# facebookresearch/multihop_dense_retrieval

Hardware: AMD Instinct MI355X
Metric: queries/sec (2-hop, beam-size x topk) over 5Mx768 index (higher is better)
Workload: dtype f32 (index stored as fp16 hi/lo pairs, fp32 accumulate); encoder f16 MFMA / f32 accumulate

## Files before the change

multihop_dense_retrieval_amd/csrc/mdr_encoder.hip:

```cpp
#include <hip/hip_runtime.h>
#include <map>
#include <mutex>
#include <algorithm>
#include <type_traits>

#include <cmath>
#include <cstdlib>
#include <cstring>
#include <new>
#include <string>
#include <vector>

#include "mdr_common.h"
#include "../../include/mdr_reader.h"

namespace mdr {
namespace {

#include "mdr_encoder_pack_ln.inl"
#include "mdr_encoder_gemm.inl"
#include "mdr_encoder_gemm_quad.inl"
#include "mdr_encoder_attention.inl"

}
}

using namespace mdr;

#ifndef MDR_CU_LANES
#define MDR_CU_LANES 0
#endif

namespace {

template <int EPI, typename C>
int launch_gemm_cfg(const _Float16* A, int lda, const _Float16* W, const float* bias, int M_cap, const int* M_dev, int N, int K, void* out, int ldo,
                    const _Float16* res, int ldr, hipStream_t st) {
    { int rc_ = ensure_dynamic_lds((const void*)gemm_f16_kernel<EPI, C>, C::LDS_BYTES); if (rc_) return rc_; }
    const int blocks = (N / C::BN) * ((M_cap + C::BM - 1) / C::BM);
    hipLaunchKernelGGL((gemm_f16_kernel<EPI, C>), dim3(blocks), dim3(C::THREADS), C::LDS_BYTES, st, A, lda, W, bias, M_cap, M_dev, N, K, out, ldo, res, ldr);
    MDR_HIP_TRY(hipGetLastError());
    return MDR_OK;
}

inline int persistent_rounds(int M_est, int bm, int N, int bn, int wgs_per_xcd) {
    const long long T = (long long)((M_est + bm - 1) / bm) * (N / bn);
    const long long per_xcd = (T + 7) / 8;
    return (int)((per_xcd + wgs_per_xcd - 1) / wgs_per_xcd);
}

template <int EPI, typename C>
int launch_gemm_persist(const _Float16* A, int lda, const _Float16* W, const float* bias, int M_cap, const int* M_dev, int N, int K, void* out, int ldo,
                        int M_est, int num_cus, hipStream_t st) {
    constexpr int lds = C::LDS_BYTES + kPersistBiasMax * 4;
    { int rc_ = ensure_dynamic_lds((const void*)gemm_persist_kernel<EPI, C>, lds); if (rc_) return rc_; }
    const int grid = num_cus / 8 * 8;
    hipLaunchKernelGGL((gemm_persist_kernel<EPI, C>), dim3(grid), dim3(C::THREADS), lds, st, A, lda, W, bias, M_cap, M_dev, N, K, out, ldo,
                       MDR_GEMM_EPI);
    MDR_HIP_TRY(hipGetLastError());
    return MDR_OK;
}

template <int EPI>
int launch_gemm_big(const _Float16* A, int lda, const _Float16* W, const float* bias, int M_cap, const int* M_dev, int N, int K, void* out, int ldo,
                    int M_est, int num_cus, hipStream_t st) {
    constexpr int lds = GemmB2::LDS_BYTES + kPersistBiasMax * 4 + 8 * 2048;
    const int grid = num_cus / 8 * 8;
    { int rc_ = ensure_dynamic_lds((const void*)gemm_big_kernel<EPI>, lds); if (rc_) return rc_; }
    hipLaunchKernelGGL((gemm_big_kernel<EPI>), dim3(grid), dim3(512), lds, st, A, lda, W, bias, M_cap, M_dev, N, K, out, ldo);
    MDR_HIP_TRY(hipGetLastError());
    return MDR_OK;
}

template <int EPI>
int launch_gemm_quad(const _Float16* A, int lda, const _Float16* W, const float* bias, int M_cap, const int* M_dev, int N, int K, void* out, int ldo,
                     int M_est, int num_cus, hipStream_t st) {
    constexpr int lds = GemmB2::LDS_BYTES + kPersistBiasMax * 4 + 4 * 4096;
    const int grid = num_cus / 8 * 8;
    { int rc_ = ensure_dynamic_lds((const void*)gemm_quad_kernel<EPI>, lds); if (rc_) return rc_; }
    hipLaunchKernelGGL((gemm_quad_kernel<EPI>), dim3(grid), dim3(256), lds, st, A, lda, W, bias, M_cap, M_dev, N, K, out, ldo);
    MDR_HIP_TRY(hipGetLastError());
    return MDR_OK;
}

template <int EPI>
int launch_gemm(const _Float16* A, int lda, const _Float16* W, const float* bias, int M_cap, const int* M_dev, int N, int K, void* out, int ldo,
                const _Float16* res, int ldr, int M_est, int num_cus, hipStream_t st, bool* res_added = nullptr, int force = -1) {
    static int env_sel = getenv("MDR_GEMM_CFG") ? atoi(getenv("MDR_GEMM_CFG")) : 0;
    int sel = force >= 0 ? force : env_sel;
    if (force < 0 && (sel == 4 || sel == 6 || sel == 7) && (long long)(N / 128) * ((M_est + 255) / 256) < (long long)num_cus * 3 / 2) sel = 0;
    if (res_added) *res_added = true;
    const long long p_tiles = (long long)(N / 128) * ((M_est + 255) / 256);
    if ((sel == 4 || sel == 6 || sel == 7 || (sel == 0 && p_tiles >= (long long)num_cus * 3 / 2)) && N % 128 == 0 && N <= kPersistBiasMax) {
        if (res_added) *res_added = false;
        else if (EPI == EPI_BIAS_RES_F32) return set_error(MDR_E_STATE, "large-M GEMM with a residual needs the caller to take the residual (res_added)");
        constexpr int E = EPI == EPI_BIAS_RES_F32 ? EPI_BIAS_F32 : EPI;
        const bool out32 = ((unsigned long long)M_cap + 255ull) * (unsigned long long)ldo * (E == EPI_BIAS_F32 ? 4ull : 2ull) < (1ull << 32);
        const bool a32 = ((unsigned long long)M_cap + 255ull) * (unsigned long long)lda * 2ull < (1ull << 32);
        if (sel == 7 && out32 && a32 && N % 256 == 0 && K % 128 == 0 && K >= 256) return launch_gemm_quad<E>(A, lda, W, bias, M_cap, M_dev, N, K, out, ldo, M_est, num_cus, st);
        if ((sel == 6 || sel == 0) && N % 256 == 0 && out32) {
            const double osz = (E == EPI_BIAS_F32) ? 4.0 : 2.0;
            const int grid = num_cus / 8 * 8, ntm_all = (M_est + 255) / 256;
            auto cost256 = [&](int max_rem, int tiles_per_pass, int* rounds_out) {
                const int head = gemm_head_row_tiles(ntm_all, N / 256, grid, max_rem);
                const int rounds = persistent_rounds(std::min(M_est, head * 256), 256, N, 256, num_cus / 8);
                const long long tail_tiles = (long long)((std::max(0, M_est - head * 256) + 127) / 128) * (N / 128);
                const long long passes = (tail_tiles + (long long)grid * tiles_per_pass - 1) / ((long long)grid * tiles_per_pass);
                if (rounds_out) *rounds_out = rounds;
                return rounds * ((256.0 + 256.0) * K * 2 + 256.0 * 256.0 * osz) + passes * 1.2 * ((128.0 + 128.0) * K * 2 + 128.0 * 128.0 * osz);
            };
            int rounds_q = 0;
            const double c_quad = cost256(grid / 4, 1, &rounds_q), c_big = cost256(grid / 2, 1, nullptr);
            const double c_p = persistent_rounds(M_est, 256, N, 128, num_cus / 8) * ((256.0 + 128.0) * K * 2 + 256.0 * 128.0 * osz);
            if (sel == 6 || std::min(c_big, c_quad) < c_p) {
                if (sel == 0 && a32 && K % 128 == 0 && K >= 256 && (rounds_q == 1 || K >= 2048) && c_quad <= 1.15 * c_big)
                    return launch_gemm_quad<E>(A, lda, W, bias, M_cap, M_dev, N, K, out, ldo, M_est, num_cus, st);
                return launch_gemm_big<E>(A, lda, W, bias, M_cap, M_dev, N, K, out, ldo, M_est, num_cus, st);
            }
        }
        return launch_gemm_persist<E, GemmP>(A, lda, W, bias, M_cap, M_dev, N, K, out, ldo, M_est, num_cus, st);
    }
    const long long big_blocks = (N % 256 == 0) ? (long long)(N / 256) * ((M_est + 255) / 256) : 0;
    const long long mid_blocks = (long long)(N / 128) * ((M_est + 127) / 128);
    const long long small_blocks = (long long)(N / 64) * ((M_est + 63) / 64);
    if (sel == 3 && big_blocks > 0) return launch_gemm_cfg<EPI, GemmBig>(A, lda, W, bias, M_cap, M_dev, N, K, out, ldo, res, ldr, st);
#ifdef MDR_GEMM_EXTRA_CFGS
    if (sel == 8) return launch_gemm_cfg<EPI, GemmCfg<128, 64, 2, 2, 3>>(A, lda, W, bias, M_cap, M_dev, N, K, out, ldo, res, ldr, st);
    if (sel == 9) return launch_gemm_cfg<EPI, GemmCfg<64, 128, 2, 2, 3>>(A, lda, W, bias, M_cap, M_dev, N, K, out, ldo, res, ldr, st);
    if (sel == 10) return launch_gemm_cfg<EPI, GemmCfg<128, 128, 2, 2, 3>>(A, lda, W, bias, M_cap, M_dev, N, K, out, ldo, res, ldr, st);
    if (sel == 11) return launch_gemm_cfg<EPI, GemmCfg<64, 64, 2, 2, 4>>(A, lda, W, bias, M_cap, M_dev, N, K, out, ldo, res, ldr, st);
    if (sel == 12) return launch_gemm_cfg<EPI, GemmCfg<128, 64, 4, 2, 3>>(A, lda, W, bias, M_cap, M_dev, N, K, out, ldo, res, ldr, st);
    if (sel == 13) return launch_gemm_cfg<EPI, GemmCfg<64, 64, 4, 2, 3>>(A, lda, W, bias, M_cap, M_dev, N, K, out, ldo, res, ldr, st);
#endif
    const long long c_mid = (mid_blocks + num_cus - 1) / num_cus * 256, c_small = (small_blocks + num_cus - 1) / num_cus * 128;
    if (N % 128 == 0 && (sel == 2 || (sel == 0 && c_mid < c_small)))
        return launch_gemm_cfg<EPI, GemmMid>(A, lda, W, bias, M_cap, M_dev, N, K, out, ldo, res, ldr, st);
    return launch_gemm_cfg<EPI, GemmSmall>(A, lda, W, bias, M_cap, M_dev, N, K, out, ldo, res, ldr, st);
}

template <int NT>
int launch_attention(const _Float16* qkv, const int* cu, int B, int L, int H, int heads, _Float16* ctx, hipStream_t st) {
    constexpr int lds = attention_lds_bytes<NT>();
    { int rc_ = ensure_dynamic_lds((const void*)attention_kernel<NT>, lds); if (rc_) return rc_; }
    dim3 grid(heads, B);
    hipLaunchKernelGGL((attention_kernel<NT>), grid, dim3(512), lds, st, qkv, cu, H, ctx);
    MDR_HIP_TRY(hipGetLastError());
    return MDR_OK;
}

int launch_attention_ring(const _Float16* qkv, const int* cu, const int* order, int B, int L, int H, int heads, _Float16* ctx, hipStream_t st) {
    { int rc_ = ensure_dynamic_lds((const void*)attention_ring_kernel, kRingLds); if (rc_) return rc_; }
    const int nblk = (L + 127) / 128;
    const long long pairs8 = ((long long)B * heads + 7) / 8 * 8;
    hipLaunchKernelGGL(attention_ring_kernel, dim3((unsigned)(pairs8 * nblk)), dim3(512), kRingLds, st, qkv, cu, order, B, heads, nblk, H, ctx);
    MDR_HIP_TRY(hipGetLastError());
    return MDR_OK;
}

template <int NTC>
int launch_attention_stream(const _Float16* qkv, const int* cu, const int* order, int B, int L, int H, int heads, _Float16* ctx, hipStream_t st) {
    if (MDR_ATTN_RING) return launch_attention_ring(qkv, cu, order, B, L, H, heads, ctx, st);
    constexpr int lds = NTC * 16 * 128 * 2;
    { int rc_ = ensure_dynamic_lds((const void*)attention_stream_kernel<NTC>, lds); if (rc_) return rc_; }
    dim3 grid(heads, B, (L + 127) / 128);
    hipLaunchKernelGGL((attention_stream_kernel<NTC>), grid, dim3(kAttnThreads), lds, st, qkv, cu, H, ctx);
    MDR_HIP_TRY(hipGetLastError());
    return MDR_OK;
}

constexpr int kOneShotMaxL = 32 * 16;
int launch_attention_for(int sel, const _Float16* qkv, const int* cu, const int* order, int B, int L, int H, int heads, _Float16* ctx, hipStream_t st) {
    if (sel == 2 || (sel == 0 && L > 128))
        return L <= 64 ? launch_attention_stream<4>(qkv, cu, order, B, L, H, heads, ctx, st) : launch_attention_stream<16>(qkv, cu, order, B, L, H, heads, ctx, st);
    if (L <= 128) return launch_attention<8>(qkv, cu, B, L, H, heads, ctx, st);
    if (L <= 384) return launch_attention<24>(qkv, cu, B, L, H, heads, ctx, st);
    return launch_attention<32>(qkv, cu, B, L, H, heads, ctx, st);
}

}

#include "mdr_encoder_trunk.inl"

struct mdr_encoder {
    Trunk t;
    _Float16* wproj = nullptr;
    float *bproj = nullptr, *lnp_g = nullptr, *lnp_b = nullptr;
    float fill_hint = 0.f;
};

namespace {

void launch_embed_ln(const long long* ids, const int* tok_src, const int* tok_pid, const int* total, int cap, const float* word, const float* pos,
                     const float* type0, const float* g, const float* b, int H, int vocab, int max_pos, float eps, _Float16* out16, float* out32,
                     hipStream_t st) {
    hipLaunchKernelGGL(embed_ln_kernel, dim3((cap + 3) / 4), dim3(256), 0, st, ids, tok_src, tok_pid, total, word, pos, type0, g, b, H, vocab, max_pos, eps,
                       out16, out32);
}

}

extern "C" {

int mdr_encoder_create(const mdr_encoder_config* cfg, const mdr_tensor* tensors, int n_tensors, int weights_on_device, int device, void* stream,
                       mdr_encoder** out) {
    MDR_REQUIRE(cfg && tensors && out, "NULL argument");
    MDR_REQUIRE(cfg->max_pos > 2, "bad geometry");
    if (int rc = trunk_check(*cfg, device)) return rc;
    DeviceGuard guard(device);
    mdr_encoder* h = new (std::nothrow) mdr_encoder();
    MDR_REQUIRE(h != nullptr, "out of host memory");
    const size_t H = cfg->hidden;
    WeightLoader ld{tensors, n_tensors, weights_on_device, (hipStream_t)stream, &h->t.allocs};
    trunk_upload(h->t, *cfg, device, 1, ld);
    ld.keep16("project.0.weight", H * H, &h->wproj);
    ld.keep32("project.0.bias", H, &h->bproj);
    ld.keep32("project.1.weight", H, &h->lnp_g);
    ld.keep32("project.1.bias", H, &h->lnp_b);
    if (int rc = ld.finish()) {
        mdr_encoder_free(h);
        return rc;
    }
    *out = h;
    return MDR_OK;
}

int mdr_test_gemm_f16(const void* A_dev, const void* W_dev, const float* bias_dev, int M, const int* m_dev, int N, int K, void* out_dev, int epilogue,
                      int kernel, int device, void* stream) {
    MDR_REQUIRE(A_dev && W_dev && bias_dev && out_dev, "NULL pointer");
    MDR_REQUIRE(M > 0 && N > 0 && K > 0 && N % 64 == 0 && K % 64 == 0, "bad GEMM shape M=%d N=%d K=%d (N, K multiples of 64)", M, N, K);
    MDR_REQUIRE(epilogue == EPI_BIAS_F16 || epilogue == EPI_BIAS_GELU_F16 || epilogue == EPI_BIAS_F32, "epilogue must be 0, 1 or 3");
#ifdef MDR_GEMM_EXTRA_CFGS
    MDR_REQUIRE(kernel == 0 || kernel == 1 || kernel == 2 || kernel == 4 || kernel == 6 || kernel == 7 || (kernel >= 8 && kernel <= 13), "kernel must be 0, 1, 2, 4, 6, 7 or 8-13");
#else
    MDR_REQUIRE(kernel == 0 || kernel == 1 || kernel == 2 || kernel == 4 || kernel == 6 || kernel == 7, "kernel must be 0, 1, 2, 4, 6 or 7");
#endif
    DeviceGuard guard(device);
    if (!guard.ok) return set_error(MDR_E_HIP, "hipSetDevice(%d) failed", device);
    const int ncu = device_cu_count(device);
    const _Float16* A = (const _Float16*)A_dev;
    const _Float16* W = (const _Float16*)W_dev;
    hipStream_t st = (hipStream_t)stream;
    if (epilogue == EPI_BIAS_F16) return launch_gemm<EPI_BIAS_F16>(A, K, W, bias_dev, M, m_dev, N, K, out_dev, N, nullptr, 0, M, ncu, st, nullptr, kernel);
    if (epilogue == EPI_BIAS_GELU_F16) return launch_gemm<EPI_BIAS_GELU_F16>(A, K, W, bias_dev, M, m_dev, N, K, out_dev, N, nullptr, 0, M, ncu, st, nullptr, kernel);
    return launch_gemm<EPI_BIAS_F32>(A, K, W, bias_dev, M, m_dev, N, K, out_dev, N, nullptr, 0, M, ncu, st, nullptr, kernel);
}

int mdr_test_gemm_ex(const void* A_dev, const void* W_dev, const float* bias_dev, const void* res16_dev, int M, int M_est, const int* m_dev, int N, int K,
                     void* out_dev, int epilogue, int kernel, int* res_added_host, int device, void* stream) {
    MDR_REQUIRE(A_dev && W_dev && bias_dev && out_dev, "NULL pointer");
    MDR_REQUIRE(M > 0 && N > 0 && K > 0 && N % 64 == 0 && K % 64 == 0, "bad GEMM shape M=%d N=%d K=%d (N, K multiples of 64)", M, N, K);
    MDR_REQUIRE(M_est >= 1, "M_est=%d must be at least 1", M_est);
    MDR_REQUIRE(epilogue >= EPI_BIAS_F16 && epilogue <= EPI_BIAS_F32, "epilogue must be 0, 1, 2 or 3");
    MDR_REQUIRE((epilogue == EPI_BIAS_RES_F32) == (res16_dev != nullptr), "res16_dev goes with epilogue 2 and with no other");
    MDR_REQUIRE(kernel == 0 || kernel == 1 || kernel == 2 || kernel == 4 || kernel == 6 || kernel == 7, "kernel must be 0, 1, 2, 4, 6 or 7");
    DeviceGuard guard(device);
    if (!guard.ok) return set_error(MDR_E_HIP, "hipSetDevice(%d) failed", device);
    const int ncu = device_cu_count(device);
    const _Float16* A = (const _Float16*)A_dev;
    const _Float16* W = (const _Float16*)W_dev;
    const _Float16* res = (const _Float16*)res16_dev;
    hipStream_t st = (hipStream_t)stream;
    bool added = true;
    bool* ra = res_added_host ? &added : nullptr;
    int rc;
    if (epilogue == EPI_BIAS_F16) rc = launch_gemm<EPI_BIAS_F16>(A, K, W, bias_dev, M, m_dev, N, K, out_dev, N, nullptr, 0, M_est, ncu, st, ra, kernel);
    else if (epilogue == EPI_BIAS_GELU_F16) rc = launch_gemm<EPI_BIAS_GELU_F16>(A, K, W, bias_dev, M, m_dev, N, K, out_dev, N, nullptr, 0, M_est, ncu, st, ra, kernel);
    else if (epilogue == EPI_BIAS_RES_F32) rc = launch_gemm<EPI_BIAS_RES_F32>(A, K, W, bias_dev, M, m_dev, N, K, out_dev, N, res, N, M_est, ncu, st, ra, kernel);
    else rc = launch_gemm<EPI_BIAS_F32>(A, K, W, bias_dev, M, m_dev, N, K, out_dev, N, nullptr, 0, M_est, ncu, st, ra, kernel);
    if (res_added_host) *res_added_host = added ? 1 : 0;
    return rc;
}

int mdr_test_attention(const void* qkv_dev, const int* cu_dev, const int* order_dev, int B, int L, int hidden, int heads, int kernel, void* ctx_dev,
                       int device, void* stream) {
    MDR_REQUIRE(qkv_dev && cu_dev && ctx_dev, "NULL pointer");
    MDR_REQUIRE(B >= 1, "B=%d must be at least 1", B);
    MDR_REQUIRE(L >= 1 && L <= 512, "L=%d out of range (1..512)", L);
    MDR_REQUIRE(heads >= 1 && hidden == 64 * heads, "head dim must be 64 (hidden=%d heads=%d)", hidden, heads);
    MDR_REQUIRE(kernel >= 0 && kernel <= 3, "kernel must be 0, 1, 2 or 3");
    MDR_REQUIRE(kernel != 1 || L <= kOneShotMaxL, "kernel 1 (one-shot) holds at most %d keys, L=%d", kOneShotMaxL, L);
    DeviceGuard guard(device);
    if (!guard.ok) return set_error(MDR_E_HIP, "hipSetDevice(%d) failed", device);
    const _Float16* qkv = (const _Float16*)qkv_dev;
    hipStream_t st = (hipStream_t)stream;
    if (kernel == 3) {
        hipLaunchKernelGGL(attention_cls_kernel, dim3(heads, B), dim3(64), 0, st, qkv, cu_dev, hidden, (_Float16*)ctx_dev);
        MDR_HIP_TRY(hipGetLastError());
        return MDR_OK;
    }
    return launch_attention_for(kernel, qkv, cu_dev, order_dev, B, L, hidden, heads, (_Float16*)ctx_dev, st);
}

#if MDR_GEMM_ABL == 5
int mdr_test_gemm_stamps(unsigned long long* out8_host, int reset) {
    MDR_REQUIRE(out8_host, "NULL pointer");
    MDR_HIP_TRY(hipDeviceSynchronize());
    MDR_HIP_TRY(hipMemcpyFromSymbol(out8_host, HIP_SYMBOL(g_gemm_stamp), 8 * sizeof(unsigned long long)));
    if (reset) {
        const unsigned long long z[8] = {0, 0, 0, 0, 0, 0, 0, 0};
        MDR_HIP_TRY(hipMemcpyToSymbol(HIP_SYMBOL(g_gemm_stamp), z, sizeof(z)));
    }
    return MDR_OK;
}
#endif

#if MDR_ATTN_ABL == 9
int mdr_test_attn_stamps(unsigned long long* out_host, int max_wgs) {
    MDR_REQUIRE(out_host && max_wgs > 0 && max_wgs <= kAttnStampWgs, "NULL pointer or max_wgs out of range");
    MDR_HIP_TRY(hipDeviceSynchronize());
    MDR_HIP_TRY(hipMemcpyFromSymbol(out_host, HIP_SYMBOL(g_attn_stamp), (size_t)max_wgs * 8 * sizeof(unsigned long long)));
    return MDR_OK;
}
#endif

#if MDR_CU_LANES
static std::mutex g_cu_mu;
static std::map<hipStream_t, int> g_stream_cus;
int mdr_stream_create_cu_range(int device, int cu_lo, int cu_hi, void** stream_out) {
    MDR_REQUIRE(stream_out != nullptr, "stream_out is NULL");
    DeviceGuard guard(device);
    if (!guard.ok) return set_error(MDR_E_HIP, "hipSetDevice(%d) failed", device);
    hipDeviceProp_t prop;
    MDR_HIP_TRY(hipGetDeviceProperties(&prop, device));
    const int n = prop.multiProcessorCount;
    MDR_REQUIRE(cu_lo >= 0 && cu_hi <= n && cu_hi - cu_lo >= 8 && cu_lo % 8 == 0 && cu_hi % 8 == 0, "CU range [%d, %d) must be multiples of 8 inside [0, %d)", cu_lo,
                cu_hi, n);
    std::vector<uint32_t> mask((size_t)(n + 31) / 32, 0u);
    for (int i = cu_lo; i < cu_hi; ++i) mask[(size_t)i / 32] |= 1u << (i % 32);
    hipStream_t st = nullptr;
    MDR_HIP_TRY(hipExtStreamCreateWithCUMask(&st, (uint32_t)mask.size(), mask.data()));
    *stream_out = (void*)st;
    return MDR_OK;
}

int mdr_stream_destroy(void* stream) {
    {
        std::lock_guard<std::mutex> lk(g_cu_mu);
        g_stream_cus.erase((hipStream_t)stream);
    }
    if (stream) MDR_HIP_TRY(hipStreamDestroy((hipStream_t)stream));
    return MDR_OK;
}
#endif

int mdr_encoder_set_fill_hint(mdr_encoder* h, float fill) {
    MDR_REQUIRE(h != nullptr, "encoder handle is NULL");
    MDR_REQUIRE(fill >= 0.f && fill <= 1.f, "fill must be in [0, 1] (0 = unknown)");
    h->fill_hint = fill;
    return MDR_OK;
}

int mdr_encoder_free(mdr_encoder* h) {
    if (!h) return MDR_OK;
    trunk_free(h->t);
    delete h;
    return MDR_OK;
}

size_t mdr_encoder_workspace_bytes(const mdr_encoder* h, int batch, int seq_len) {
    if (!h || batch <= 0 || seq_len <= 0) return 0;
    return carve(h->t.cfg, batch, seq_len, nullptr).bytes;
}

int mdr_encoder_forward(mdr_encoder* h, const int64_t* ids_dev, const int64_t* mask_dev, int batch, int seq_len, float* out_dev, void* workspace_dev,
                        size_t workspace_bytes, void* stream) {
    MDR_REQUIRE(h != nullptr, "encoder handle is NULL");
    MDR_REQUIRE(batch >= 0 && seq_len > 0, "bad shape batch=%d seq_len=%d", batch, seq_len);
    if (batch == 0) return MDR_OK;
    MDR_REQUIRE(ids_dev && mask_dev && out_dev, "NULL pointer");
    MDR_REQUIRE(seq_len <= 512, "seq_len=%d exceeds 512 (RoBERTa has 514 positions)", seq_len);
    MDR_REQUIRE((long long)batch * seq_len < (1ll << 31), "batch*seq_len overflows int32; split the batch");
    const Trunk& t = h->t;
    const mdr_encoder_config& c = t.cfg;
    DeviceGuard guard(t.device);
    hipStream_t st = (hipStream_t)stream;
    const long long* ids = (const long long*)ids_dev;
    Workspace w;
    if (int rc = trunk_begin(t, ids, (const long long*)mask_dev, batch, seq_len, workspace_dev, workspace_bytes, carve(c, batch, seq_len, nullptr).bytes, st, &w))
        return rc;
    const int B = batch, L = seq_len, H = c.hidden;
    const int Tcap = B * L;
    const int Test = h->fill_hint > 0.f ? std::max(1, (int)(h->fill_hint * (float)Tcap)) : Tcap - Tcap / 3;
    int ncu = t.num_cus;
#if MDR_CU_LANES
    {
        std::lock_guard<std::mutex> lk(g_cu_mu);
        auto it = g_stream_cus.find(st);
        if (it != g_stream_cus.end()) ncu = it->second;
        else {
            uint32_t mask[32] = {0};
            int n = 0;
            hipStreamCaptureStatus cs = hipStreamCaptureStatusNone;
            if (hipStreamIsCapturing(st, &cs) == hipSuccess && cs == hipStreamCaptureStatusNone && hipExtStreamGetCUMask(st, 32, mask) == hipSuccess)
                for (uint32_t w_ : mask) n += __builtin_popcount(w_);
            else (void)hipGetLastError();
            if (n >= 8 && n < t.num_cus) ncu = n / 8 * 8;
            if (cs == hipStreamCaptureStatusNone) g_stream_cus[st] = ncu;
        }
    }
#endif
    launch_embed_ln(ids, w.tok_src, w.tok_pid, w.total, Tcap, t.word, t.pos, t.type, t.emb_g, t.emb_b, H, c.vocab, c.max_pos, c.ln_eps, w.h16, w.h32, st);
    MDR_HIP_TRY(hipGetLastError());
    const Rows tokens{w.h16, w.h32, w.pre, Tcap, w.total, Test}, cls{w.cls16, w.cls32, w.clspre, B, nullptr, B};
    int rc;
    for (int i = 0; i + 1 < c.layers; ++i) {
        rc = trunk_layer(t, t.layers[i], w, tokens, B, L, ncu, st);
        if (rc) return rc;
    }
    const Layer& last = t.layers.back();
    rc = launch_qkv(t, last, w, tokens, ncu, st);
    if (rc) return rc;
    launch_gather_cls(w.h16, w.h32, w.cu, B, H, w.cls16, w.cls32, st);
    hipLaunchKernelGGL(attention_cls_kernel, dim3(c.heads, B), dim3(64), 0, st, (const _Float16*)w.qkv, (const int*)w.cu, H, w.ctx);
    MDR_HIP_TRY(hipGetLastError());
    rc = layer_tail(t, last, w.ctx, w.ffn, cls, ncu, st);
    if (rc) return rc;
    rc = launch_gemm<EPI_BIAS_F32>(w.cls16, H, h->wproj, h->bproj, B, nullptr, H, H, w.clspre, H, nullptr, 0, B, ncu, st);
    if (rc) return rc;
    launch_layernorm((const float*)w.clspre, (const _Float16*)nullptr, (const float*)nullptr, B, (const int*)nullptr, H, h->lnp_g, h->lnp_b, c.ln_eps,
                     (_Float16*)nullptr, out_dev, st);
    MDR_HIP_TRY(hipGetLastError());
    return MDR_OK;
}

}

#include "mdr_reader.inl"
#include "mdr_reader_assemble.inl"
#include "mdr_encoder_test_rows.inl"
#include "mdr_linear_grad.inl"
```

Measured before the change: 14830.

## Compute last-layer Q only for CLS rows and add tiny-M GEMM path

In the final encoder layer, only K and V are projected for all tokens. Q is computed just for the gathered CLS rows through a separate small GEMM, and the CLS attention kernel takes a separate Q pointer and stride. This removes the Q third of the last layer's QKV projection across all tokens. A GemmTiny configuration is also selected automatically for very small M. The diff references launch_kv, w.qcls, GemmTiny and kGemmSelTiny, none of which are defined in the visible changes, so it depends on edits to other files.

```diff
diff --git a/include/mdr_encoder_tail.h b/include/mdr_encoder_tail.h
--- /dev/null
+++ b/include/mdr_encoder_tail.h
@@ -0,0 +1,17 @@
+#ifndef MDR_ENCODER_TAIL_H
+#define MDR_ENCODER_TAIL_H
+
+#include "mdr_hip.h"
+
+#ifdef __cplusplus
+extern "C" {
+#endif
+
+int mdr_test_attention_cls(const void* q_dev, const void* qkv_dev, const int* cu_dev, int B, int hidden, int heads, void* ctx_dev, int device,
+                           void* stream);
+
+#ifdef __cplusplus
+}
+#endif
+
+#endif
diff --git a/multihop_dense_retrieval_amd/csrc/mdr_encoder.hip b/multihop_dense_retrieval_amd/csrc/mdr_encoder.hip
--- a/multihop_dense_retrieval_amd/csrc/mdr_encoder.hip
+++ b/multihop_dense_retrieval_amd/csrc/mdr_encoder.hip
@@ -13,6 +13,7 @@
 
 #include "mdr_common.h"
 #include "../../include/mdr_reader.h"
+#include "../../include/mdr_encoder_tail.h"
 
 namespace mdr {
 namespace {
@@ -120,6 +121,8 @@
         }
         return launch_gemm_persist<E, GemmP>(A, lda, W, bias, M_cap, M_dev, N, K, out, ldo, M_est, num_cus, st);
     }
+    if ((sel == kGemmSelTiny || (sel == 0 && M_cap <= kGemmTinyMaxRows && M_est <= kGemmTinyMaxRows)) && K % (BK * GemmTiny::KSUB) == 0)
+        return launch_gemm_cfg<EPI, GemmTiny>(A, lda, W, bias, M_cap, M_dev, N, K, out, ldo, res, ldr, st);
     const long long big_blocks = (N % 256 == 0) ? (long long)(N / 256) * ((M_est + 255) / 256) : 0;
     const long long mid_blocks = (long long)(N / 128) * ((M_est + 127) / 128);
     const long long small_blocks = (long long)(N / 64) * ((M_est + 63) / 64);
@@ -164,6 +167,13 @@
     { int rc_ = ensure_dynamic_lds((const void*)attention_stream_kernel<NTC>, lds); if (rc_) return rc_; }
     dim3 grid(heads, B, (L + 127) / 128);
     hipLaunchKernelGGL((attention_stream_kernel<NTC>), grid, dim3(kAttnThreads), lds, st, qkv, cu, H, ctx);
+    MDR_HIP_TRY(hipGetLastError());
+    return MDR_OK;
+}
+
+int launch_attention_cls(const _Float16* q, int ldq, int q_by_cu, const _Float16* qkv, const int* cu, int B, int H, int heads, _Float16* ctx_cls,
+                         hipStream_t st) {
+    hipLaunchKernelGGL(attention_cls_kernel, dim3(heads, B), dim3(64), 0, st, q, ldq, q_by_cu, qkv, cu, H, ctx_cls);
     MDR_HIP_TRY(hipGetLastError());
     return MDR_OK;
 }
@@ -252,7 +262,8 @@
     MDR_REQUIRE(M_est >= 1, "M_est=%d must be at least 1", M_est);
     MDR_REQUIRE(epilogue >= EPI_BIAS_F16 && epilogue <= EPI_BIAS_F32, "epilogue must be 0, 1, 2 or 3");
     MDR_REQUIRE((epilogue == EPI_BIAS_RES_F32) == (res16_dev != nullptr), "res16_dev goes with epilogue 2 and with no other");
-    MDR_REQUIRE(kernel == 0 || kernel == 1 || kernel == 2 || kernel == 4 || kernel == 6 || kernel == 7, "kernel must be 0, 1, 2, 4, 6 or 7");
+    MDR_REQUIRE(kernel == 0 || kernel == 1 || kernel == 2 || kernel == 4 || kernel == 6 || kernel == 7 || kernel == kGemmSelTiny,
+                "kernel must be 0, 1, 2, 4, 6, 7 or 16");
     DeviceGuard guard(device);
     if (!guard.ok) return set_error(MDR_E_HIP, "hipSetDevice(%d) failed", device);
     const int ncu = device_cu_count(device);
@@ -283,12 +294,20 @@
     if (!guard.ok) return set_error(MDR_E_HIP, "hipSetDevice(%d) failed", device);
     const _Float16* qkv = (const _Float16*)qkv_dev;
     hipStream_t st = (hipStream_t)stream;
-    if (kernel == 3) {
-        hipLaunchKernelGGL(attention_cls_kernel, dim3(heads, B), dim3(64), 0, st, qkv, cu_dev, hidden, (_Float16*)ctx_dev);
-        MDR_HIP_TRY(hipGetLastError());
-        return MDR_OK;
-    }
+    if (kernel == 3)
+        return launch_attention_cls(qkv, 3 * hidden, 1, qkv, cu_dev, B, hidden, heads, (_Float16*)ctx_dev, st);
     return launch_attention_for(kernel, qkv, cu_dev, order_dev, B, L, hidden, heads, (_Float16*)ctx_dev, st);
+}
+
+int mdr_test_attention_cls(const void* q_dev, const void* qkv_dev, const int* cu_dev, int B, int hidden, int heads, void* ctx_dev, int device,
+                           void* stream) {
+    MDR_REQUIRE(q_dev && qkv_dev && cu_dev && ctx_dev, "NULL pointer");
+    MDR_REQUIRE(B >= 1, "B=%d must be at least 1", B);
+    MDR_REQUIRE(heads >= 1 && hidden == 64 * heads, "head dim must be 64 (hidden=%d heads=%d)", hidden, heads);
+    DeviceGuard guard(device);
+    if (!guard.ok) return set_error(MDR_E_HIP, "hipSetDevice(%d) failed", device);
+    return launch_attention_cls((const _Float16*)q_dev, hidden, 0, (const _Float16*)qkv_dev, cu_dev, B, hidden, heads, (_Float16*)ctx_dev,
+                                (hipStream_t)stream);
 }
 
 #if MDR_GEMM_ABL == 5
@@ -408,11 +427,14 @@
         if (rc) return rc;
     }
     const Layer& last = t.layers.back();
-    rc = launch_qkv(t, last, w, tokens, ncu, st);
+    rc = launch_kv(t, last, w, tokens, ncu, st);
     if (rc) return rc;
     launch_gather_cls(w.h16, w.h32, w.cu, B, H, w.cls16, w.cls32, st);
-    hipLaunchKernelGGL(attention_cls_kernel, dim3(c.heads, B), dim3(64), 0, st, (const _Float16*)w.qkv, (const int*)w.cu, H, w.ctx);
-    MDR_HIP_TRY(hipGetLastError());
+    MDR_HIP_TRY(hipGetLastError());
+    rc = launch_gemm<EPI_BIAS_F16>(w.cls16, H, last.wqkv, last.bqkv, B, nullptr, H, H, w.qcls, H, nullptr, 0, B, ncu, st);
+    if (rc) return rc;
+    rc = launch_attention_cls(w.qcls, H, 0, w.qkv, w.cu, B, H, c.heads, w.ctx, st);
+    if (rc) return rc;
     rc = layer_tail(t, last, w.ctx, w.ffn, cls, ncu, st);
     if (rc) return rc;
     rc = launch_gemm<EPI_BIAS_F32>(w.cls16, H, h->wproj, h->bproj, B, nullptr, H, H, w.clspre, H, nullptr, 0, B, ncu, st);
```

New measurement: 14970, median of 6. No clear change (+0.9%).
